# ZHANGKEON/DIS-YOLO

Hardware: AMD Instinct MI355X
Metric: train images/sec @576x576 bf16 (higher is better)
Workload: dtype bf16

## Files before the change

dis-yolo_amd/csrc/conv_igemm.hip:

```cpp
#include <utility>
#include "common.h"
#include "conv_common.h"
#include "runtime.h"

using namespace dyconv;

namespace {

template <int BM, int BN, int WM, int WN, int BK, int ST, int KS, int KG = 1, int EPI = 0>
__global__ __launch_bounds__(WM* WN * 64 * KG, (BM == 128 && BN == 128) ? 3 : 1) void conv_igemm_kernel(ConvParams p) {
#ifdef HALO_PROBE
  long long gp_t[5];
  gp_t[0] = (long long)__builtin_amdgcn_s_memtime();
  gp_t[4] = (long long)__builtin_amdgcn_s_memrealtime();
#endif
  constexpr int NW = WM * WN;
  constexpr int T = NW * 64;
  constexpr int WTM = BM / WM, WTN = BN / WN;
  constexpr int MI = WTM / 16, NI = WTN / 16;
  constexpr int ROWB = BK * 2;
  constexpr int CPR = ROWB / 16;
  constexpr int SLAB = 1024 * NW;
  constexpr int A_BYTES = (BM * ROWB + SLAB - 1) / SLAB * SLAB;
  constexpr int B_BYTES = (BN * ROWB + SLAB - 1) / SLAB * SLAB;
// ... 1421 lines not shown
          v[0] += __builtin_bit_cast(float, rr.x << 16);
          v[1] += __builtin_bit_cast(float, rr.x & 0xffff0000u);
          v[2] += __builtin_bit_cast(float, rr.y << 16);
          v[3] += __builtin_bit_cast(float, rr.y & 0xffff0000u);
        }
        uint2 o2;
        o2.x = pack2(v[0], v[1]);
        o2.y = pack2(v[2], v[3]);
        *reinterpret_cast<uint2*>(sw + (t * 16 + frow) * ROWP + (j * 16 + cq * 4) * 2) = o2;
      }
    }
    __builtin_amdgcn_fence(__ATOMIC_RELEASE, "wavefront");
    __builtin_amdgcn_wave_barrier();
    __builtin_amdgcn_fence(__ATOMIC_ACQUIRE, "wavefront");
#pragma unroll
    for (int t = 0; t < FW; ++t) {
#pragma unroll
      for (int r_ = 0; r_ < RPF; ++r_) {
        const int idx = r_ * 64 + lane;
        const int r16 = idx / CPR8, ch = idx % CPR8;
        const int m = __shfl(m_of[t], r16, 64);
        const int n = n0 + ch * 8;
        const uint4 o = *reinterpret_cast<const uint4*>(sw + (t * 16 + r16) * ROWP + ch * 16);
        unsigned off = (m >= 0 && n < p.Cout) ? (unsigned)(((size_t)m * p.Cout + n) * 2) : OOB;
#ifdef DY_PROBE
        if (p.flags & 0x80000) off = OOB;
#endif
        buffer_store16(o, off, srdy);
      }
    }
  }
}

template <int NI>
__global__ __launch_bounds__(512) void conv1x1_stream_kernel(ConvParams p, int ngroups) {
  constexpr int NW = 8, U = 2;
  constexpr int BN = NI * 16;
  constexpr int ROWP = BN * 2 + 16;
  constexpr int STG = U * 16 * ROWP;
  constexpr int MAXKS = 6;
  extern __shared__ __attribute__((aligned(16))) char smem[];
  const int tid = threadIdx.x;
  const int lane = tid & 63;
  const int wave = __builtin_amdgcn_readfirstlane(tid >> 6);
  const int frow = lane & 15, cq = lane >> 4;
  const int K = p.K, ks32 = K >> 5;
  const int wpitch = K * 2 + 16;
  char* const wl = smem;
  char* const stg = smem + ((BN * wpitch + 15) & ~15);
  for (int c = tid; c < BN * (K >> 3); c += NW * 64) {
    const int n = c / (K >> 3), kc = c - n * (K >> 3);
    uint4 v = uint4{0, 0, 0, 0};
    if (n < p.Cout) v = *reinterpret_cast<const uint4*>(p.w + (size_t)n * K + kc * 8);
    *reinterpret_cast<uint4*>(wl + n * wpitch + kc * 16) = v;
  }
  float esc[NI][4], esh[NI][4];
#pragma unroll
  for (int j = 0; j < NI; ++j)
#pragma unroll
    for (int r = 0; r < 4; ++r) {
      const int n = j * 16 + cq * 4 + r;
      esc[j][r] = (p.scale && n < p.Cout) ? p.scale[n] : 1.f;
      esh[j][r] = (p.shift && n < p.Cout) ? p.shift[n] : 0.f;
    }
  __syncthreads();
  const bool f32out = p.flags & DISYOLO_CONV_OUT_F32;
  const bool do_stats = p.flags & DISYOLO_CONV_STATS;
  const bool vec_ok = (p.Cout & 7) == 0;
  const bool use_res = p.residual != nullptr;
  const int H1 = p.H >> 1, W1 = p.W >> 1;
  const int ks0 = p.C0 >> 5;
  float s1[NI][4], s2[NI][4];
#pragma unroll
  for (int j = 0; j < NI; ++j)
#pragma unroll
    for (int r = 0; r < 4; ++r) s1[j][r] = s2[j][r] = 0.f;
  char* const sw = stg + wave * STG;

  for (int g = blockIdx.x * NW + wave; g < ngroups; g += gridDim.x * NW) {
    int m_of[U];
    bf16x8 xf[U][MAXKS];
#pragma unroll
    for (int u = 0; u < U; ++u) {
      const int m = g * (U * 16) + u * 16 + frow;
      m_of[u] = m < p.M ? m : -1;
      const int mm = m < p.M ? m : 0;
      const bf16* a0 = p.x0 + (size_t)mm * p.C0 + cq * 8;
      const bf16* a1 = a0;
      if (p.C1 > 0) {
        int b, rem, y, x;
        divmod_small(mm, p.H * p.W, b, rem);
        divmod_small(rem, p.W, y, x);
        a1 = p.x1 + ((size_t)(b * H1 + (y >> 1)) * W1 + (x >> 1)) * p.C1 + cq * 8;
      }
#pragma unroll
      for (int k = 0; k < MAXKS; ++k)
        if (k < ks32) xf[u][k] = *reinterpret_cast<const bf16x8*>(k < ks0 ? a0 + k * 32 : a1 + (k - ks0) * 32);
    }
    uint2 rres[U][NI];
    if (use_res) {
#pragma unroll
      for (int u = 0; u < U; ++u)
#pragma unroll
        for (int j = 0; j < NI; ++j) {
          const int n = j * 16 + cq * 4;
          rres[u][j] = *reinterpret_cast<const uint2*>(p.residual + (size_t)(m_of[u] >= 0 ? m_of[u] : 0) * p.Cout + (n + 3 < p.Cout ? n : 0));
        }
    }
    f32x4 acc[U][NI];
#pragma unroll
    for (int u = 0; u < U; ++u)
#pragma unroll
      for (int j = 0; j < NI; ++j) acc[u][j] = f32x4{0.f, 0.f, 0.f, 0.f};
#pragma unroll
    for (int k = 0; k < MAXKS; ++k) {
      if (k < ks32) {
        bf16x8 wf[NI];
#pragma unroll
        for (int j = 0; j < NI; ++j) wf[j] = *reinterpret_cast<const bf16x8*>(wl + (j * 16 + frow) * wpitch + (k * 4 + cq) * 16);
#pragma unroll
        for (int u = 0; u < U; ++u)
#pragma unroll
          for (int j = 0; j < NI; ++j) acc[u][j] = __builtin_amdgcn_mfma_f32_16x16x32_bf16(wf[j], xf[u][k], acc[u][j], 0, 0, 0);
      }
    }
    if (do_stats) {
#pragma unroll
      for (int u = 0; u < U; ++u)
#pragma unroll
        for (int j = 0; j < NI; ++j)
// ... 155 lines not shown
  static bool attr_set = false;
  if (!attr_set) {
    (void)hipFuncSetAttribute(reinterpret_cast<const void*>(&conv_stream_kernel<NW, FW, NI>),
                              hipFuncAttributeMaxDynamicSharedMemorySize, (int)lds);
    attr_set = true;
  }
  static const int ncu = [] {
    int dev = 0, n = 256;
    if (hipGetDevice(&dev) == hipSuccess) (void)hipDeviceGetAttribute(&n, hipDeviceAttributeMultiprocessorCount, dev);
    return n > 0 ? n : 256;
  }();
  int G = ncu / q.tilesN;
  if (G < 1) G = 1;
  if (G > q.tilesM) G = q.tilesM;
  hipLaunchKernelGGL((conv_stream_kernel<NW, FW, NI>), dim3(G * q.tilesN), dim3(NW * 64), lds, s, q, pt.ph, pt.pw, tilesY,
                     tilesX, G);
  DY_CHECK_LAUNCH();
  return DISYOLO_OK;
}

bool stream1x1_ok(const disyolo_conv_desc* d) {
  if (d->ksize != 1 || d->stride != 1 || d->in_div != 1 || d->Ho != d->H || d->Wo != d->W) return false;
  if (d->Cout > 64 || d->C0 % 32 || d->C1 % 32 || d->C0 + d->C1 > 192) return false;
  if (d->flags & DISYOLO_CONV_BN_BWD_STATS) return false;
  return true;
}
int stream1x1_blocks(int M) {
  const int groups = ceil_div(M, 32);
  int blocks = ceil_div(groups, 8 * 4);
  if (blocks > 512) blocks = 512;
  if (blocks < 1) blocks = 1;
  return blocks;
}
template <int NI>
int launch_stream1x1_n(const ConvParams& p, hipStream_t s) {
  constexpr int BN = NI * 16;
  const size_t wbytes = ((size_t)BN * (p.K * 2 + 16) + 15) & ~(size_t)15;
  const size_t lds = wbytes + (size_t)8 * 2 * 16 * (BN * 2 + 16) + (size_t)8 * BN * 8;
  static bool attr_set = false;
  if (!attr_set) {
    (void)hipFuncSetAttribute(reinterpret_cast<const void*>(&conv1x1_stream_kernel<NI>), hipFuncAttributeMaxDynamicSharedMemorySize,
                              (int)(64 * (192 * 2 + 16) + 8 * 2 * 16 * (64 * 2 + 16) + 8 * 64 * 8));
    attr_set = true;
  }
  hipLaunchKernelGGL((conv1x1_stream_kernel<NI>), dim3(stream1x1_blocks(p.M)), dim3(512), lds, s, p, ceil_div(p.M, 32));
  DY_CHECK_LAUNCH();
  return DISYOLO_OK;
}
int launch_stream1x1(const ConvParams& p, hipStream_t s) {
  if (p.Cout <= 16) return launch_stream1x1_n<1>(p, s);
  if (p.Cout <= 32) return launch_stream1x1_n<2>(p, s);
  return launch_stream1x1_n<4>(p, s);
}

struct LaunchQuery {
  bool active = false, have = false, want_bwd = false, want_fused = false;
  int grid = 0, rows = 0, bn = 0, resident = 0;
};
thread_local LaunchQuery tl_query;
template <class K>
int resident_blocks(K kernel, int threads, size_t lds) {
  int dev = 0, cus = 0, occ = 0;
  if (hipGetDevice(&dev) != hipSuccess) return 0;
  if (hipDeviceGetAttribute(&cus, hipDeviceAttributeMultiprocessorCount, dev) != hipSuccess) return 0;
  if (hipOccupancyMaxActiveBlocksPerMultiprocessor(&occ, reinterpret_cast<const void*>(kernel), threads, lds) != hipSuccess) {
    (void)hipGetLastError();
    return 0;
  }
  const int by_lds = lds ? (int)((size_t)160 * 1024 / lds) : 8;
  const int by_waves = 32 / (threads / 64);
  if (occ > by_lds) occ = by_lds;
  if (occ > by_waves) occ = by_waves;
  return occ * cus;
}

template <int NW, int FW, int NI>
int launch_halo(const ConvParams& p, Patch pt, hipStream_t s) {
  ConvParams q = p;
  constexpr int BN = NI * 16;
  const int tilesY = p.H / pt.ph, tilesX = p.W / pt.pw;
  q.tilesM = p.B * tilesY * tilesX;
  q.tilesN = ceil_div(p.Cout, BN);
  q.xcd_n = (q.tilesN >= 8 && (int64_t)p.bytesw > (int64_t)p.bytes0) ? 1 : 0;
  q.halo_split = 1;
  constexpr int SLAB = NW * 1024, BIM = (9 * BN * 4 + NW * 64 - 1) / (NW * 64);
// ... 364 lines not shown
extern "C" int disyolo_dgrad_s2_quad_ok(int B, int Hdy, int Wdy, int Cdy, int C) {
  return (B > 0 && Hdy > 0 && Wdy > 0 && Cdy % 64 == 0 && C % 8 == 0 && (4 * C) % 128 == 0 && C <= 64 &&
          (int64_t)B * Hdy * Wdy * 4 * C * 2 < (1LL << 31) && (int64_t)B * Hdy * Wdy * Cdy * 2 < (1LL << 31)) ? 1 : 0;
}

extern "C" int disyolo_dgrad_s2_quad(const void* dy, const void* wq, void* dx, const void* residual, int B, int Hdy, int Wdy,
                                     int Cdy, int C, void* stream) {
  DY_REQUIRE(dy && wq && dx, "dgrad_s2_quad: null pointer");
  DY_REQUIRE(disyolo_dgrad_s2_quad_ok(B, Hdy, Wdy, Cdy, C) == 1, "dgrad_s2_quad: needs Cdy %% 64 == 0, C in {32, 64}");
  DY_RECORD_OR_RUN([=](void* s) { return disyolo_dgrad_s2_quad(dy, wq, dx, residual, B, Hdy, Wdy, Cdy, C, s); });
  ConvParams p;
  p.x0 = (const bf16*)dy; p.x1 = nullptr; p.w = (const bf16*)wq;
  p.scale = nullptr; p.shift = nullptr; p.residual = (const bf16*)residual; p.y = dx; p.stats = nullptr;
  p.bn_x = nullptr; p.bn_scale = p.bn_shift = p.bn_mean = p.bn_rstd = nullptr; p.bn_part = nullptr; p.bn_alpha = 0.f;
  p.B = B; p.H = Hdy; p.W = Wdy; p.C0 = Cdy; p.C1 = 0; p.Cin = Cdy;
  p.Ho = Hdy; p.Wo = Wdy; p.Cout = 4 * C;
  p.ks = 3; p.stride = 1; p.pad_t = 1; p.pad_l = 1; p.dmask = 0; p.dshift = 0;
  p.M = B * Hdy * Wdy;
  p.K = 9 * Cdy;
  p.bytes0 = (unsigned)((size_t)B * Hdy * Wdy * Cdy * 2);
  p.bytes1 = 0;
  p.bytesw = (unsigned)((size_t)4 * C * 9 * Cdy * 2);
  p.nk = 0;
  p.flags = 0;
  p.alpha = 0.f;
  p.tilesM = p.tilesN = 0;
  p.xcd_n = 0; p.halo_split = 0;
  p.pcls = 0; p.Mc = 0; p.tilesMc = 0;
  p.tapmask = 0x1b;
  p.d2s_c = C;
  return launch<192, 128, 4, 2, 64, 2>(p, (hipStream_t)stream);
}

static int conv2d_fwd_core(const disyolo_conv_desc* d, void* stream);

extern "C" int disyolo_cluster_sync_words(int Cout) { return Cout > 0 ? (ceil_div(Cout, 16) + 1) * CL_LINE : 0; }

extern "C" int disyolo_cluster_sync_error(const uint32_t* cluster_sync, int Cout) {
  if (!cluster_sync || Cout <= 0) return 0;
  uint32_t w = 0;
  if (hipMemcpy(&w, cluster_sync + (size_t)ceil_div(Cout, 16) * CL_LINE, sizeof(w), hipMemcpyDeviceToHost) != hipSuccess) {
    (void)hipGetLastError();
    return -1;
  }
  return (int)w;
}

extern "C" int disyolo_conv2d_bn_fused_ok(const disyolo_conv_desc* d) {
  if (!d || validate(d) != DISYOLO_OK) return 0;
  if ((d->flags & DISYOLO_CONV_OUT_F32) || d->Cout % 8) return 0;
  if (d->in_div != 1 && (d->flags & (DISYOLO_CONV_STATS | DISYOLO_CONV_BN_FUSED))) return 0;
  static const bool on = [] { const char* e = getenv("DISYOLO_BN_INKERNEL"); return !(e && e[0] == '0'); }();
  if (!on) return 0;
  tl_query = LaunchQuery{};
  tl_query.active = true;
  tl_query.want_bwd = (d->flags & DISYOLO_CONV_BN_BWD_FUSED) != 0;
  tl_query.want_fused = true;
  disyolo_conv_desc c = *d;
  c.flags &= ~(DISYOLO_CONV_BN_FUSED | DISYOLO_CONV_BN_BWD_FUSED | DISYOLO_CONV_BN_BWD_STATS);
  const int rc = conv2d_fwd_core(&c, nullptr);
  const LaunchQuery q = tl_query;
  tl_query = LaunchQuery{};
  if (rc != DISYOLO_OK || !q.have) return 0;
  if ((int64_t)q.rows * q.bn * 8 > 128 * 1024) return 0;
  return (q.resident > 0 && q.grid <= q.resident) ? 1 : 0;
}

extern "C" int disyolo_conv2d_fwd(const disyolo_conv_desc* d, void* stream) {
  int rc = validate(d);
  if (rc) return rc;
  DY_REQUIRE(!(d->flags & DISYOLO_CONV_STATS) || d->stats, "conv: STATS flag without stats buffer");
  if (d->flags & DISYOLO_CONV_BN_FUSED) {
    DY_REQUIRE((d->flags & DISYOLO_CONV_STATS) && !(d->flags & (DISYOLO_CONV_LEAKY | DISYOLO_CONV_OUT_F32 | DISYOLO_CONV_BN_BWD_STATS)) &&
                   !d->scale && !d->shift && !d->residual && d->Cout % 8 == 0,
               "conv: BN_FUSED needs STATS, bf16 y, no scale / shift / LEAKY / residual (y is the raw conv output), Cout %% 8 == 0");
    DY_REQUIRE(d->y_act && d->bn_gamma && d->bn_beta && d->bn_out_scale && d->bn_out_shift && d->bn_out_mean && d->bn_out_rstd &&
                   d->cluster_sync, "conv: BN_FUSED with a null y_act / bn_gamma / bn_beta / bn_out_* / cluster_sync");
  }
  if (d->flags & DISYOLO_CONV_BN_BWD_FUSED) {
    DY_REQUIRE((d->flags & DISYOLO_CONV_BN_BWD_STATS) && d->bn_dgamma && d->bn_dbeta && d->cluster_sync,
               "conv: BN_BWD_FUSED needs BN_BWD_STATS (the bn_* fields) and bn_dgamma / bn_dbeta / cluster_sync");
  }
  {
    const disyolo_conv_desc c = *d;
    DY_RECORD_OR_RUN([c](void* s) { return disyolo_conv2d_fwd(&c, s); });
  }
  return conv2d_fwd_core(d, stream);
}

static int conv2d_fwd_core(const disyolo_conv_desc* d, void* stream) {
  if (conv_c16_shape(d)) {
    if (tl_query.active) return DISYOLO_OK;
    return conv_c16_launch(d, stream);
  }
  ConvParams p;
  p.x0 = (const bf16*)d->x0;
  p.x1 = (const bf16*)d->x1;
  p.w = (const bf16*)d->w;
  p.scale = d->scale;
  p.shift = d->shift;
  p.residual = (const bf16*)d->residual;
  p.y = d->y;
  p.stats = d->stats;
  p.bn_x = nullptr; p.bn_scale = p.bn_shift = p.bn_mean = p.bn_rstd = nullptr; p.bn_part = nullptr; p.bn_alpha = 0.f;
  if (d->flags & DISYOLO_CONV_BN_BWD_STATS) {
    DY_REQUIRE(d->bn_x && d->bn_scale && d->bn_shift && d->bn_mean && d->bn_rstd && d->bn_partials,
               "conv: BN_BWD_STATS flag with a null bn_* pointer");
    DY_REQUIRE((d->flags & DISYOLO_CONV_BN_BWD_FUSED) || disyolo_conv2d_bn_bwd_stats_ok(d) == 1,
               "conv: BN_BWD_STATS needs a patch kernel (tile 16-19, 24, 25 on a shape it covers) or a GEMM tile with that epilogue "
               "(ask disyolo_conv2d_bn_bwd_stats_ok), bf16 output, Cout %% 8 == 0");
    DY_REQUIRE(!(d->flags & DISYOLO_CONV_BN_BWD_FUSED) || (!(d->flags & (DISYOLO_CONV_OUT_F32 | DISYOLO_CONV_STATS | DISYOLO_CONV_LEAKY)) &&
                                                          !d->scale && !d->shift && d->Cout % 8 == 0),
               "conv: BN_BWD_FUSED needs a plain bf16 data-gradient conv (no scale / shift / LEAKY / STATS), Cout %% 8 == 0");
    p.bn_x = (const bf16*)d->bn_x; p.bn_scale = d->bn_scale; p.bn_shift = d->bn_shift; p.bn_mean = d->bn_mean;
    p.bn_rstd = d->bn_rstd; p.bn_part = d->bn_partials; p.bn_alpha = d->bn_alpha;
  }
  p.B = d->B; p.H = d->H; p.W = d->W; p.C0 = d->C0; p.C1 = d->C1; p.Cin = d->C0 + d->C1;
  p.Ho = d->Ho; p.Wo = d->Wo; p.Cout = d->Cout;
  p.ks = d->ksize; p.stride = d->stride; p.pad_t = d->pad_t; p.pad_l = d->pad_l;
  p.dmask = d->in_div - 1; p.dshift = d->in_div == 2 ? 1 : 0;
  p.M = d->B * d->Ho * d->Wo;
  p.K = d->ksize * d->ksize * p.Cin;
  p.bytes0 = (unsigned)((size_t)d->B * d->H * d->W * d->C0 * 2);
  p.bytes1 = (unsigned)((size_t)d->B * (d->H / 2) * (d->W / 2) * d->C1 * 2);
  p.bytesw = (unsigned)((size_t)d->Cout * p.K * 2);
  p.nk = 0;
  p.flags = d->flags;
  p.alpha = d->alpha;
  p.tilesM = p.tilesN = 0;
  p.xcd_n = 0; p.halo_split = 0;
  p.pcls = 0; p.Mc = 0; p.tilesMc = 0;
  p.tapmask = 0; p.d2s_c = 0;
  p.y_act = d->y_act; p.gamma = d->bn_gamma; p.beta = d->bn_beta; p.mm = d->bn_moving_mean; p.mv = d->bn_moving_var;
  p.o_scale = d->bn_out_scale; p.o_shift = d->bn_out_shift; p.o_mean = d->bn_out_mean; p.o_rstd = d->bn_out_rstd;
  p.dgamma = d->bn_dgamma; p.dbeta = d->bn_dbeta; p.csync = d->cluster_sync;
  p.bn_decay = d->bn_decay; p.bn_eps = d->bn_eps; p.inv_count = 1.0 / (double)p.M;
  hipStream_t s = (hipStream_t)stream;
  Patch pt;
  const int sel = resolve_sel(d, p.M, &pt);
  {
    const int id = sel & 0xff;
    if (id == 24 || id == 25 || id == 20 || id == 21) {
      if (tl_query.active) return DISYOLO_OK;
      DY_REQUIRE(!(d->flags & (DISYOLO_CONV_BN_FUSED | DISYOLO_CONV_BN_BWD_FUSED)),
                 "conv: BN_FUSED / BN_BWD_FUSED on a tile whose kernel has no such epilogue (ask disyolo_conv2d_bn_fused_ok)");
    }
  }
  switch (sel & 0xff) {
    case 24:
    case 25: return launch_flat(p, sel & 0xff, s);
#ifndef DY_ONLY_HALO
    case 21: return launch_stream1x1(p, s);
    case 20: return launch_stream(p, pt, s);
#endif
    case 16: return launch_halo<8, 3, 4>(p, pt, s);
    case 18: return launch_halo<8, 3, 2>(p, pt, s);
    case 19: return launch_halo<8, 3, 1>(p, pt, s);
    case 17: return launch_halo<4, 3, 4>(p, pt, s);
    default: break;
  }
  const bool bk64 = (d->C0 % 64 == 0) && (d->C1 % 64 == 0) && !(sel & 0x100);
  return dispatch(sel & 0xff, bk64, (sel >> 9) & 1, p, s);
}
```

dis-yolo_amd/lib.py:

```python
from __future__ import annotations

import ctypes as C
import os
from typing import Optional

import numpy as np
import torch

_HERE = os.path.dirname(os.path.abspath(__file__))
LIB_PATH = os.environ.get("DISYOLO_LIB", os.path.join(_HERE, "libdisyolo_hip.so"))

GRAD_LD = 32
ROI_MAX = 16
ROI_W = 12
K_MAPS = (3, 5, 7)
MASK_STRIDES = (1, 2, 4)


def roi_w(k: int) -> int:
    return 2 * (k + 1) + 4


def block32_post(k: int) -> int:
    return {3: 1, 5: 2, 7: 3}[k]
# ... 8 lines not shown
    _fields_ = [
        ("B", C.c_int32), ("H", C.c_int32), ("W", C.c_int32),
        ("C0", C.c_int32), ("C1", C.c_int32),
        ("Ho", C.c_int32), ("Wo", C.c_int32), ("Cout", C.c_int32),
        ("ksize", C.c_int32), ("stride", C.c_int32),
        ("pad_t", C.c_int32), ("pad_l", C.c_int32),
        ("in_div", C.c_int32), ("flags", C.c_int32),
        ("alpha", C.c_float), ("tile", C.c_int32),
        ("x0", C.c_void_p), ("x1", C.c_void_p), ("w", C.c_void_p),
        ("scale", C.c_void_p), ("shift", C.c_void_p), ("residual", C.c_void_p),
        ("y", C.c_void_p), ("stats", C.c_void_p),
        ("bn_x", C.c_void_p), ("bn_scale", C.c_void_p), ("bn_shift", C.c_void_p), ("bn_mean", C.c_void_p),
        ("bn_rstd", C.c_void_p), ("bn_partials", C.c_void_p), ("bn_alpha", C.c_float),
        ("bn_decay", C.c_float), ("bn_eps", C.c_float),
        ("y_act", C.c_void_p), ("bn_gamma", C.c_void_p), ("bn_beta", C.c_void_p),
        ("bn_moving_mean", C.c_void_p), ("bn_moving_var", C.c_void_p),
        ("bn_out_scale", C.c_void_p), ("bn_out_shift", C.c_void_p), ("bn_out_mean", C.c_void_p), ("bn_out_rstd", C.c_void_p),
        ("bn_dgamma", C.c_void_p), ("bn_dbeta", C.c_void_p), ("cluster_sync", C.c_void_p),
    ]


_SIGS = {
    "disyolo_version": (C.c_int, []),
    "disyolo_last_error": (C.c_char_p, []),
    "disyolo_conv_desc_size": (C.c_size_t, []),
    "disyolo_find_contours": (C.c_int, [C.c_void_p, C.c_int, C.c_int, C.c_void_p, C.c_int64, C.c_void_p, C.c_void_p, C.c_int,
                                        C.POINTER(C.c_int), C.POINTER(C.c_int64)]),
    "disyolo_conv2d_stats_rows": (C.c_int, [C.POINTER(ConvDesc)]),
    "disyolo_conv2d_bn_bwd_stats_ok": (C.c_int, [C.POINTER(ConvDesc)]),
    "disyolo_conv2d_bn_fused_ok": (C.c_int, [C.POINTER(ConvDesc)]),
    "disyolo_cluster_sync_words": (C.c_int, [C.c_int]),
    "disyolo_cluster_sync_error": (C.c_int, [C.c_void_p, C.c_int]),
    "disyolo_conv2d_fwd": (C.c_int, [C.POINTER(ConvDesc), C.c_void_p]),
    "disyolo_conv2d_tile": (C.c_int, [C.POINTER(ConvDesc)] + [C.POINTER(C.c_int)] * 4),
    "disyolo_conv_first_fwd": (C.c_int, [C.c_void_p] * 5 + [C.c_int] * 4 + [C.c_float, C.c_void_p]),
    "disyolo_conv12_fused_ok": (C.c_int, [C.c_int] * 3),
    "disyolo_conv12_fused_fwd": (C.c_int, [C.c_void_p] * 8 + [C.c_int] * 3 + [C.c_float, C.c_void_p]),
    "disyolo_block32_fused_ok": (C.c_int, [C.c_int] * 6),
    "disyolo_block64_fused_ok": (C.c_int, [C.c_int] * 4),
    "disyolo_pack_quad": (C.c_int, [C.c_void_p, C.c_void_p, C.c_int, C.c_int, C.c_void_p]),
    "disyolo_dgrad_s2_quad_ok": (C.c_int, [C.c_int] * 5),
    "disyolo_dgrad_s2_quad": (C.c_int, [C.c_void_p] * 4 + [C.c_int] * 5 + [C.c_void_p]),
    "disyolo_block64_fused_fwd": (C.c_int, [C.c_void_p] * 8 + [C.c_int] * 4 + [C.c_float, C.c_void_p]),
    "disyolo_block32_fused_fwd": (C.c_int, [C.c_void_p, C.c_void_p, C.c_int, C.c_int] + [C.c_void_p] * 6 + [C.c_int] +
                                  [C.c_void_p] * 3 + [C.c_int] * 3 + [C.c_float, C.c_void_p]),
    "disyolo_conv2d_wgrad_workspace": (C.c_size_t, [C.POINTER(ConvDesc), C.c_int]),
    "disyolo_conv2d_wgrad": (C.c_int, [C.POINTER(ConvDesc), C.c_void_p, C.c_int, C.c_void_p, C.c_void_p,
                                       C.c_size_t, C.c_int, C.c_void_p]),
    "disyolo_conv2d_fp8_fwd": (C.c_int, [C.POINTER(ConvDesc), C.c_void_p, C.c_void_p, C.c_void_p, C.c_void_p, C.c_float,
                                         C.c_void_p, C.c_float, C.c_void_p, C.c_void_p]),
    "disyolo_conv_first_fwd_fp8": (C.c_int, [C.c_void_p] * 5 + [C.c_float] + [C.c_int] * 4 + [C.c_float, C.c_void_p]),
    "disyolo_quant_fp8": (C.c_int, [C.c_void_p, C.c_int, C.c_void_p, C.c_int64, C.c_float, C.c_void_p]),
    "disyolo_dequant_fp8": (C.c_int, [C.c_void_p, C.c_void_p, C.c_int64, C.c_float, C.c_void_p]),
    "disyolo_pack_weights_fp8": (C.c_int, [C.c_void_p, C.c_void_p] + [C.c_int] * 3 + [C.c_float, C.c_void_p]),
    "disyolo_conv2d_wgrad_plan": (C.c_int, [C.POINTER(ConvDesc), C.c_int] + [C.POINTER(C.c_int)] * 4),
    "disyolo_conv_first_wgrad_workspace": (C.c_size_t, [C.c_int] * 4),
    "disyolo_conv_first_wgrad": (C.c_int, [C.c_void_p] * 3 + [C.c_int] * 4 + [C.c_void_p, C.c_size_t, C.c_void_p]),
    "disyolo_image_pad8": (C.c_int, [C.c_void_p, C.c_void_p, C.c_int64, C.c_void_p]),
    "disyolo_copy2d_f32": (C.c_int, [C.c_void_p, C.c_void_p] + [C.c_int] * 4 + [C.c_void_p]),
    "disyolo_pack_weights": (C.c_int, [C.c_void_p] * 3 + [C.c_int] * 4 + [C.c_void_p]),
    "disyolo_pack_table_bytes": (C.c_size_t, [C.c_int]),
    "disyolo_pack_table_build": (C.c_int, [C.c_void_p, C.c_int, C.c_void_p, C.POINTER(C.c_int)]),
    "disyolo_pack_all": (C.c_int, [C.c_void_p, C.c_int, C.c_int, C.c_void_p]),
    "disyolo_bn_finalize": (C.c_int, [C.c_void_p, C.c_int, C.c_int, C.c_int64] + [C.c_void_p] * 4 +
                            [C.c_float, C.c_float] + [C.c_void_p] * 5),
    "disyolo_colstats_rows": (C.c_int, [C.c_int64, C.c_int]),
# ... 406 lines not shown
def conv2d_tile(d: ConvDesc):
    bm, bn, bk, st = C.c_int(0), C.c_int(0), C.c_int(0), C.c_int(0)
    tid = load().disyolo_conv2d_tile(C.byref(d), C.byref(bm), C.byref(bn), C.byref(bk), C.byref(st))
    if tid < 0:
        raise DisyoloError("conv2d_tile: bad descriptor")
    return tid, bm.value, bn.value, bk.value, st.value


def conv2d_fwd(d: ConvDesc) -> None:
    if TUNER is not None:
        TUNER.launch(d)
        return
    if TIMER is not None:
        if not hasattr(d, "_tname"):
            tid, bm, bn, bk, st = conv2d_tile(d)
            if tid in (24, 25):
                d._tname = "conv_flat_kernel<%s,2,%d>" % ("2,3,2,1" if tid == 24 else "4,3,1,2", st)
            elif tid == 21:
                d._tname = "conv1x1_stream_kernel<%d>" % (bn // 16)
            elif tid == 20:
                d._tname = "conv_stream_kernel<8,3,4>"
            elif tid >= 16:
                d._tname = "conv_halo_kernel<%d,3,%d>" % (4 if tid == 17 else 8, 2 if tid == 18 else 1 if tid == 19 else 4)
            else:
                d._tname = "conv_igemm_kernel<%d,%d,%d,%d,%d,%d,%d,%d,%d>" % ((bm, bn) + _WAVES.get(tid, (0, 0)) +
                                                                               (bk, st, d.ksize, 2 if 13 <= tid <= 15 else 1,
                                                                                1 if d.flags & CONV_BN_BWD_FUSED else 0))
        TIMER.run(d._tname, conv_flops(d), lambda: _check(load().disyolo_conv2d_fwd(C.byref(d), _stream()),
                                                           "conv2d_fwd"), conv_bytes(d))
        return
    _check(load().disyolo_conv2d_fwd(C.byref(d), _stream()), "conv2d_fwd")


def conv2d_fp8_fwd(d: ConvDesc, w8, escale, eshift, y8, out_scale: float, y16=None, residual8=None,
                   residual_scale: float = 0.0) -> None:
    if TIMER is not None:
        name = "conv_fp8_kernel<%d,%d,3>" % (128 if d.Cout > 64 else (64 if d.Cout > 32 else 32), 64 if d.C0 % 64 == 0 else 32)
        TIMER.run(name, conv_flops(d), lambda: _check(load().disyolo_conv2d_fp8_fwd(
            C.byref(d), _p(w8), _p(escale), _p(eshift), _p(residual8), residual_scale, _p(y8), out_scale, _p(y16), _stream()),
            "conv2d_fp8_fwd"))
        return
    _check(load().disyolo_conv2d_fp8_fwd(C.byref(d), _p(w8), _p(escale), _p(eshift), _p(residual8), residual_scale, _p(y8),
                                         out_scale, _p(y16), _stream()), "conv2d_fp8_fwd")


def conv_first_fwd_fp8(images, w_hwio, scale, shift, y8, out_scale: float, alpha=0.1) -> None:
    _need(images, torch.float32, "images")
    _need(y8, torch.uint8, "y8")
    B, H, W, _ = images.shape
    _check(load().disyolo_conv_first_fwd_fp8(_p(images), _p(w_hwio), _p(scale), _p(shift), _p(y8), out_scale, B, H, W,
                                             y8.shape[-1], alpha, _stream()), "conv_first_fwd_fp8")


def quant_fp8(x, y8, scale: float) -> None:
    if x.dtype not in (torch.bfloat16, torch.float32) or not x.is_contiguous():
        raise DisyoloError("quant_fp8: x must be contiguous bf16 or f32")
    _check(load().disyolo_quant_fp8(_p(x), int(x.dtype == torch.float32), _p(y8), x.numel(), scale, _stream()), "quant_fp8")


def dequant_fp8(x8, y, scale: float) -> None:
    _need(y, torch.float32, "y")
    _check(load().disyolo_dequant_fp8(_p(x8), _p(y), x8.numel(), scale, _stream()), "dequant_fp8")


def pack_weights_fp8(w_hwio, w8, ksize, cin, cout, scale: float) -> None:
    _check(load().disyolo_pack_weights_fp8(_p(w_hwio), _p(w8), ksize, cin, cout, scale, _stream()), "pack_weights_fp8")
# ... 595 lines not shown
```

dis-yolo_amd/net.py:

```python
from __future__ import annotations

from typing import Dict, List, Optional, Sequence, Tuple

import math
import json
import contextlib
import os
import sys
import numpy as np
import torch

from . import config as cfg
from . import lib as L

BF16 = torch.bfloat16
F32 = torch.float32

WGRAD_GROUP = 3
OPT_CHUNK_ELEMS = 8_000_000
PIPE_LANE = 2


class Layer:
    __slots__ = ("idx", "cin", "cout", "k", "stride", "kind", "src", "src_up", "shortcut", "lock", "H", "W", "Ho",
                 "Wo", "w", "bias", "gamma", "beta", "mm", "mv", "scale", "shift", "mean", "rstd", "wp", "wdg", "raw",
                 "act", "stats", "stats_rows", "desc", "grad", "grad_set", "need_grad", "dw", "dbias", "dgamma",
                 "dbeta", "dx", "pad_t", "pad_l", "dgrad_descs", "wgrad_desc", "cout_pad",
                 "act8", "w8", "s_w", "s_out", "escale", "desc8", "dual16", "bn_sums", "bwd_local", "bwd_global", "bwd_part", "bwd_part_rows", "wq",
                 "csync", "fused_fwd", "csync_bwd", "fused_bwd", "passthru")

    def __init__(self, idx, cin, cout, k, stride, kind, src, src_up=None, shortcut=None):
        self.idx, self.cin, self.cout, self.k, self.stride, self.kind = idx, cin, cout, k, stride, kind
        self.src, self.src_up, self.shortcut = src, src_up, shortcut
        for s in self.__slots__[9:]:
            setattr(self, s, None)


MASK_STRIDES = (4, 2, 1)


def build_topology(num_class: int, k_map: int, mask_stride: int = 2) -> List[Layer]:
    if mask_stride not in MASK_STRIDES:
        raise ValueError("mask_stride must be one of %s (got %r)" % (", ".join(map(str, MASK_STRIDES)), mask_stride))
    out_depth = (num_class + 5) * 3
    Ls: List[Layer] = []

    def add(idx, cin, cout, k, s, kind, src, src_up=None, shortcut=None):
        Ls.append(Layer(idx, cin, cout, k, s, kind, src, src_up, shortcut))

    add(1, 3, 32, 3, 1, "bn", 0)
    add(2, 32, 64, 3, 2, "bn", 1)
    i = 3
    ch = 64
    for nblocks, down in ((1, 5), (2, 10), (8, 27), (8, 44), (4, None)):
        for _ in range(nblocks):
            add(i, ch, ch // 2, 1, 1, "bn", i - 1)
            add(i + 1, ch // 2, ch, 3, 1, "res", i, shortcut=i - 1)
            i += 2
        if down:
            add(down, ch, ch * 2, 3, 2, "bn", down - 1)
            ch *= 2
            i = down + 1
# ... 99 lines not shown
            self.ws = L.Workspace(self.device)
            self.ws_aux = L.Workspace(self.device)
            self.ws_det = L.Workspace(self.device)
        self._reg_fresh = False
        self.lock = {i: (stage == 1 and i <= 52) for i in range(1, self.score_layer + 1)}
        for i, v in (lock or {}).items():
            if isinstance(i, bool) or not isinstance(i, (int, np.integer)) or not 1 <= i <= self.score_layer:
                raise ValueError("lock: %r is not a layer of this net (1..%d)" % (i, self.score_layer))
            self.lock[int(i)] = bool(v)
        self.layers = build_topology(self.num_class, self.k, self.mask_stride)
        self.by_idx = {l.idx: l for l in self.layers}
        self._mark_pass_through()
        if self.dtype == "fp8":
            self._check_fp8_lock()
        self._lr = float(cfg.LEARNING_RATE)
        self.lr_dev = None
        self.dp = None
        self.sync_bn = False
        self._rec = None
        self._prog = None
        self._prog_marks = []
        self._graph = None
        self.opt_chunks = None
        self._overlap = False
        self._overlap_rec = False
        self._tail_open = False
        self._progs = None
        self.fuse_first_two = True
        self.fuse_blocks = True
        self.use_side_lane = os.environ.get("DISYOLO_SIDE_LANE", "1") != "0"
        self.bn_inkernel = os.environ.get("DISYOLO_BN_INKERNEL", "1") != "0"
        self.bn_inkernel_bwd = os.environ.get("DISYOLO_BN_INKERNEL_BWD", "0") == "1"
        self.bn_fuse_check = None
        self.tail_on_main = 0
        self.pair = bool(backbone_pair)
        self._half = 0
        self._pair_P = 0
        self._init_params(seed, xavier_locked)
        if self.pair:
            if not self.training or self.dtype != "bf16" or self.plan_only:
                raise L.DisyoloError("backbone_pair needs a bf16 training net")
            self._pair_P = self._backbone_prefix()
            if self._pair_P < 2:
                raise L.DisyoloError("backbone_pair needs a locked layer prefix (stage 1)")
        if not self.plan_only:
            self._plan(self.batchsize, self.image_size)

    def _init_params(self, seed: int, xavier_locked: bool) -> None:
        dev = self.device
        g = torch.Generator().manual_seed(seed)
        n_decay = 0
        n_nodecay = 0
        for l in self.layers:
            l.lock = self.lock[l.idx]
            if not l.lock:
                n_decay += l.k * l.k * l.cin * l.cout + (l.cout if l.kind == "lin" else 0)
                if l.kind != "lin":
                    n_nodecay += 2 * l.cout
        self.n_decay, self.n_params = n_decay, n_decay + n_nodecay
        n = max(self.n_params, 1)
        self.arena = torch.zeros(n, dtype=F32, device=dev)
        self.grad_arena = torch.zeros(n, dtype=F32, device=dev)
        self.adam_m = torch.zeros(n, dtype=F32, device=dev)
        self.adam_v = torch.zeros(n, dtype=F32, device=dev)
        self.step_dev = torch.zeros(1, dtype=torch.int64, device=dev)
        self.lr_dev = torch.full((1,), self._lr, dtype=F32, device=dev)
# ... 283 lines not shown
            if l.kind == "lin":
                l.desc = L.make_conv_desc(x0, l.wp, l.act, l.k, l.stride, x1=x1, shift=l.bias, out_f32=True)
            elif train_bn:
                if l.stats is None:
                    d0 = L.make_conv_desc(x0, l.wp, l.raw, l.k, l.stride, x1=x1)
                    l.stats_rows = L.conv2d_stats_rows(d0)
                    l.stats = torch.zeros(l.stats_rows, l.cout, 2, dtype=F32, device=dev)
                l.desc = L.make_conv_desc(x0, l.wp, l.raw, l.k, l.stride, x1=x1, stats=l.stats)
                l.fused_fwd = False
                if (self.bn_inkernel and not self.sync_bn and res is None and l.idx not in self.HEAD_LAYERS
                        and not getattr(self, "plan_only", False) and l.stride == 1):
                    tile = self._fused_tile(lambda t: L.make_conv_desc(x0, l.wp, l.raw, l.k, l.stride, x1=x1, tile=t), l.k)
                    if tile is not None:
                        d0 = L.make_conv_desc(x0, l.wp, l.raw, l.k, l.stride, x1=x1, tile=tile)
                        rows = L.conv2d_stats_rows(d0)
                        l.stats_rows = rows
                        if l.stats.shape[0] < rows:
                            l.stats = torch.zeros(rows, l.cout, 2, dtype=F32, device=dev)
                        if l.csync is None:
                            l.csync = L.cluster_sync_buffer(l.cout, dev)
                        l.desc = L.make_conv_desc(x0, l.wp, l.raw, l.k, l.stride, x1=x1, stats=l.stats, tile=tile,
                                                  bn_fused=dict(y_act=l.act, gamma=l.gamma, beta=l.beta, mm=l.mm, mv=l.mv,
                                                                scale=l.scale, shift=l.shift, mean=l.mean, rstd=l.rstd,
                                                                decay=cfg.BN_DECAY, eps=cfg.BN_EPSILON, sync=l.csync),
                                                  alpha=cfg.ALPHA)
                        l.fused_fwd = True
            elif l.passthru:
                l.desc = L.make_conv_desc(x0, l.wp, l.raw, l.k, l.stride, x1=x1)
            else:
                l.desc = L.make_conv_desc(x0, l.wp, l.act, l.k, l.stride, x1=x1, scale=l.scale, shift=l.shift,
                                          residual=res, leaky=True, alpha=cfg.ALPHA)
            if self.training and not l.lock:
                l.wgrad_desc = L.make_conv_desc(x0, l.wp, l.act, l.k, l.stride, x1=x1)

    FUSED_TILES_1x1 = (3, 2, 6, 10, 1, 12, 0x20c)
    FUSED_TILES_3x3 = (16, 18, 19, 12, 0x20c)

    def _fused_tile(self, make_desc, k: int, bwd: bool = False):
        best, best_blocks = None, -1
        for i, t in enumerate((0,) + (self.FUSED_TILES_3x3 if k == 3 else self.FUSED_TILES_1x1)):
            d = make_desc(t)
            tid, bm, bn, _, _ = L.conv2d_tile(d)
            if t and tid != (t & 0xff):
                continue
            if bwd:
                d.flags |= L.CONV_BN_BWD_FUSED
            ok = L.conv2d_bn_fused_ok(d)
            d.flags &= ~L.CONV_BN_BWD_FUSED
            if not ok:
                continue
            if i == 0:
                return d.tile
            blocks = L.conv2d_stats_rows(d) * (-(-d.Cout // bn))
            if blocks > best_blocks:
                best, best_blocks = t, blocks
        return best

    def _input_of(self, l, src: int) -> torch.Tensor:
        a = self.by_idx[src].act
        if self.pair and src <= self._pair_P < l.idx:
            return a[self._half * self.B:(self._half + 1) * self.B]
        return a

    def _backbone_prefix(self) -> int:
        p = 0
        for l in self.layers:
# ... 262 lines not shown
                    and L.block32_fused_ok(self.B, l82.Ho, l82.Wo, self.by_idx[l80.src].cout, self.by_idx[l80.src_up].cout,
                                           L.block32_post(self.k))):
                plan[80], plan[81], plan[82] = None, None, self._forward_mask_head
        return plan

    def _can_fuse_first_two(self, is_training: bool) -> bool:
        if not self.fuse_first_two or (self.dtype == "fp8" and self.fp8_ready and self.FP8_FROM <= 2):
            return False
        if not self._inference_mode((1, 2), is_training):
            return False
        if any(1 in (l.src, l.src_up, l.shortcut) for l in self.layers if l.idx != 2):
            return False
        return L.conv12_fused_ok(self.B, self.S, self.S)

    def _forward_layer(self, l, is_training: bool) -> None:
        B = self.B
        if self.dtype == "fp8" and self.fp8_ready and l.act8 is not None and l.idx >= self.FP8_FROM:
            self._forward_layer_fp8(l)
            return
        train_bn = is_training and self.training and (not l.lock) and l.kind != "lin"
        M = B * l.Ho * l.Wo
        res = self._input_of(l, l.shortcut) if l.shortcut is not None else None
        if l.idx == 1:
            if train_bn:
                L.conv_first_fwd(self.images, l.w, self._ones32, self._zeros32, l.raw, alpha=1.0)
                L.colstats(l.raw, l.stats, M, l.cout)
                self._bn_finalize(l, M)
                L.bn_act_fwd(l.raw, l.scale, l.shift, None, l.act, M, l.cout, cfg.ALPHA)
            else:
                if not l.lock and self.training:
                    L.bn_fold(l.gamma, l.beta, l.mm, l.mv, cfg.BN_EPSILON, l.scale, l.shift)
                L.conv_first_fwd(self.images, l.w, l.scale, l.shift, l.act, alpha=cfg.ALPHA)
            return
        if l.kind == "lin":
            L.conv2d_fwd(l.desc)
        elif l.passthru and is_training:
            L.conv2d_fwd(l.desc)
            L.bn_act_fwd(l.raw, l.scale, l.shift, res, l.act, M, l.cout, cfg.ALPHA)
        elif train_bn:
            L.conv2d_fwd(l.desc)
            if l.fused_fwd and L.TUNER is None:
                return
            self._bn_finalize(l, M)
            L.bn_act_fwd(l.raw, l.scale, l.shift, res, l.act, M, l.cout, cfg.ALPHA)
        else:
            if self.training and (not l.lock or l.passthru):
                if not l.lock:
                    L.bn_fold(l.gamma, l.beta, l.mm, l.mv, cfg.BN_EPSILON, l.scale, l.shift)
                d = L.make_conv_desc(self._input_of(l, l.src), l.wp, l.act, l.k, l.stride,
                                     x1=self._input_of(l, l.src_up) if l.src_up is not None else None,
                                     scale=l.scale, shift=l.shift, residual=res, leaky=True, alpha=cfg.ALPHA)
                L.conv2d_fwd(d)
            else:
                L.conv2d_fwd(l.desc)

    def _bn_finalize(self, l, M: int) -> None:
        rows = l.stats_rows
        if L.TUNER is not None:
            rows = L.TUNER.stats_rows.get(l.stats.data_ptr(), rows)
        if not self.sync_bn:
            L.bn_finalize(l.stats, rows, l.cout, M, l.gamma, l.beta, l.mm, l.mv, cfg.BN_DECAY,
                          cfg.BN_EPSILON, l.scale, l.shift, l.mean, l.rstd)
            return
        L.bn_partial_sums(l.stats, rows, l.cout, l.bn_sums)
        self._sync_sums(l.bn_sums)
        L.bn_finalize_sums(l.bn_sums, l.cout, M * self.dp.world_size, l.gamma, l.beta, l.mm, l.mv, cfg.BN_DECAY,
                           cfg.BN_EPSILON, l.scale, l.shift, l.mean, l.rstd)

    def _sync_sums(self, t: torch.Tensor) -> None:
        if self.dp.inlist:
            self.dp.comm.allreduce(t)
        elif self._rec is not None:
            prog, marks = self._rec
            marks.append((prog.size(), ("sync", t, L.CURRENT_LANE)))
        else:
            import torch.distributed as dist
# ... 826 lines not shown
```

include/disyolo.h:

```cpp
#ifndef DISYOLO_H
#define DISYOLO_H

#include <stddef.h>
#include <stdint.h>

#ifdef __cplusplus
extern "C" {
#endif

#define DISYOLO_OK 0
#define DISYOLO_E_ARG (-1)
#define DISYOLO_E_WORKSPACE (-2)
#define DISYOLO_E_HIP (-3)

#define DISYOLO_GRAD_LD 32
#define DISYOLO_ROI_MAX 16
#define DISYOLO_ROI_W 12
#define DISYOLO_ROI_W_K(k) (2 * ((k) + 1) + 4)

int disyolo_version(void);
const char* disyolo_last_error(void);

enum {
  DISYOLO_CONV_LEAKY = 1,
// ... 24 lines not shown
  float* stats;
  const void* bn_x;
  const float* bn_scale;
  const float* bn_shift;
  const float* bn_mean;
  const float* bn_rstd;
  float* bn_partials;
  float bn_alpha;
  float bn_decay, bn_eps;
  void* y_act;
  const float* bn_gamma;
  const float* bn_beta;
  float* bn_moving_mean;
  float* bn_moving_var;
  float* bn_out_scale;
  float* bn_out_shift;
  float* bn_out_mean;
  float* bn_out_rstd;
  float* bn_dgamma;
  float* bn_dbeta;
  uint32_t* cluster_sync;
} disyolo_conv_desc;

int disyolo_find_contours(const uint8_t* binary, int h, int w, int32_t* points_xy, int64_t max_points,
                          int32_t* contour_start, int32_t* hierarchy, int max_contours, int* n_contours,
                          int64_t* n_points);
size_t disyolo_conv_desc_size(void);
int disyolo_conv2d_bn_bwd_stats_ok(const disyolo_conv_desc* d);
int disyolo_conv2d_bn_fused_ok(const disyolo_conv_desc* d);
int disyolo_cluster_sync_words(int Cout);
int disyolo_cluster_sync_error(const uint32_t* cluster_sync, int Cout);
int disyolo_conv2d_stats_rows(const disyolo_conv_desc* d);
int disyolo_conv2d_fwd(const disyolo_conv_desc* d, void* stream);
int disyolo_conv2d_tile(const disyolo_conv_desc* d, int* bm, int* bn, int* bk, int* stages);

int disyolo_conv_first_fwd(const float* images, const float* w_hwio, const float* scale,
                           const float* shift, void* y_bf16, int B, int H, int W, int Cout,
                           float alpha, void* stream);

int disyolo_conv12_fused_ok(int B, int H, int W);
int disyolo_conv12_fused_fwd(const float* images, const float* w1_hwio, const float* scale1, const float* shift1,
                             const void* w2_packed, const float* scale2, const float* shift2, void* y_bf16, int B, int H,
                             int W, float alpha, void* stream);

int disyolo_block32_fused_ok(int B, int H, int W, int C0, int C1, int post);
int disyolo_block32_fused_fwd(const void* x0, const void* x1, int C0, int C1, const void* wA, const float* scaleA,
                              const float* shiftA, const void* wB, const float* scaleB, const float* shiftB, int post,
                              const void* wC, const float* biasC, void* y, int B, int H, int W, float alpha, void* stream);

int disyolo_block64_fused_ok(int B, int H, int W, int C0);
int disyolo_block64_fused_fwd(const void* x, const void* wA, const float* scaleA, const float* shiftA, const void* wB,
                              const float* scaleB, const float* shiftB, void* y, int B, int H, int W, int C0, float alpha,
                              void* stream);

int disyolo_pack_quad(const float* w_hwio, void* wq, int C, int Cdy, void* stream);
int disyolo_dgrad_s2_quad_ok(int B, int Hdy, int Wdy, int Cdy, int C);
int disyolo_dgrad_s2_quad(const void* dy, const void* wq, void* dx, const void* residual, int B, int Hdy, int Wdy, int Cdy,
                          int C, void* stream);

enum {
  DISYOLO_WGRAD_IM2COL = 1,
  DISYOLO_WGRAD_PARTIAL_ONLY = 2,
  DISYOLO_WGRAD_REDUCE_ONLY = 4,
  DISYOLO_WGRAD_STAGES_MASK = 0x30
};
size_t disyolo_conv2d_wgrad_workspace(const disyolo_conv_desc* d, int opts);
// ... 218 lines not shown
```

Measured before the change: 2148.

## Fuse producer BN+leaky activation into streaming 1x1 conv input load

Adds a BNL variant of the streaming 1x1 conv kernel. It reads the producer layer's raw pre-BN output, applies the producer's batch-norm scale/shift and leaky activation on load, and writes the activated tensor out for backward use. The network planner finds eligible producer→1x1 consumer pairs and skips the separate bn_act_fwd launch for those producers. This removes a kernel launch and one read of the raw tensor per pair. In exchange the consumer kernel does extra ALU work, extra stores and a little more LDS.

```diff
diff --git a/dis-yolo_amd/csrc/conv_igemm.hip b/dis-yolo_amd/csrc/conv_igemm.hip
--- a/dis-yolo_amd/csrc/conv_igemm.hip
+++ b/dis-yolo_amd/csrc/conv_igemm.hip
@@ -1477,7 +1477,7 @@
   }
 }
 
-template <int NI>
+template <int NI, bool BNL = false>
 __global__ __launch_bounds__(512) void conv1x1_stream_kernel(ConvParams p, int ngroups) {
   constexpr int NW = 8, U = 2;
   constexpr int BN = NI * 16;
@@ -1499,6 +1499,13 @@
     if (n < p.Cout) v = *reinterpret_cast<const uint4*>(p.w + (size_t)n * K + kc * 8);
     *reinterpret_cast<uint4*>(wl + n * wpitch + kc * 16) = v;
   }
+  float* const isc = reinterpret_cast<float*>(stg + NW * STG + NW * BN * 8);
+  if (BNL) {
+    for (int c = tid; c < p.C0; c += NW * 64) {
+      isc[c] = p.bn_scale[c];
+      isc[p.C0 + c] = p.bn_shift[c];
+    }
+  }
   float esc[NI][4], esh[NI][4];
 #pragma unroll
   for (int j = 0; j < NI; ++j)
@@ -1541,6 +1548,28 @@
 #pragma unroll
       for (int k = 0; k < MAXKS; ++k)
         if (k < ks32) xf[u][k] = *reinterpret_cast<const bf16x8*>(k < ks0 ? a0 + k * 32 : a1 + (k - ks0) * 32);
+    }
+    if (BNL) {
+#pragma unroll
+      for (int k = 0; k < MAXKS; ++k) {
+        if (k < ks32) {
+          const int c0 = k * 32 + cq * 8;
+          const float4 s0 = *reinterpret_cast<const float4*>(isc + c0), s1 = *reinterpret_cast<const float4*>(isc + c0 + 4);
+          const float4 h0 = *reinterpret_cast<const float4*>(isc + p.C0 + c0), h1 = *reinterpret_cast<const float4*>(isc + p.C0 + c0 + 4);
+          const float sc[8] = {s0.x, s0.y, s0.z, s0.w, s1.x, s1.y, s1.z, s1.w};
+          const float sh[8] = {h0.x, h0.y, h0.z, h0.w, h1.x, h1.y, h1.z, h1.w};
+#pragma unroll
+          for (int u = 0; u < U; ++u) {
+            float v[8];
+            unpack8(__builtin_bit_cast(uint4, xf[u][k]), v);
+#pragma unroll
+            for (int e = 0; e < 8; ++e) v[e] = leaky(v[e] * sc[e] + sh[e], p.bn_alpha);
+            const uint4 o = pack8(v);
+            xf[u][k] = __builtin_bit_cast(bf16x8, o);
+            if (m_of[u] >= 0) *reinterpret_cast<uint4*>(reinterpret_cast<bf16*>(p.y_act) + (size_t)m_of[u] * p.C0 + c0) = o;
+          }
+        }
+      }
     }
     uint2 rres[U][NI];
     if (use_res) {
@@ -1762,25 +1791,26 @@
   if (blocks < 1) blocks = 1;
   return blocks;
 }
-template <int NI>
+template <int NI, bool BNL = false>
 int launch_stream1x1_n(const ConvParams& p, hipStream_t s) {
   constexpr int BN = NI * 16;
   const size_t wbytes = ((size_t)BN * (p.K * 2 + 16) + 15) & ~(size_t)15;
-  const size_t lds = wbytes + (size_t)8 * 2 * 16 * (BN * 2 + 16) + (size_t)8 * BN * 8;
+  const size_t lds = wbytes + (size_t)8 * 2 * 16 * (BN * 2 + 16) + (size_t)8 * BN * 8 + (BNL ? (size_t)p.C0 * 8 : 0);
   static bool attr_set = false;
   if (!attr_set) {
-    (void)hipFuncSetAttribute(reinterpret_cast<const void*>(&conv1x1_stream_kernel<NI>), hipFuncAttributeMaxDynamicSharedMemorySize,
-                              (int)(64 * (192 * 2 + 16) + 8 * 2 * 16 * (64 * 2 + 16) + 8 * 64 * 8));
+    (void)hipFuncSetAttribute(reinterpret_cast<const void*>(&conv1x1_stream_kernel<NI, BNL>), hipFuncAttributeMaxDynamicSharedMemorySize,
+                              (int)(64 * (192 * 2 + 16) + 8 * 2 * 16 * (64 * 2 + 16) + 8 * 64 * 8 + 192 * 8));
     attr_set = true;
   }
-  hipLaunchKernelGGL((conv1x1_stream_kernel<NI>), dim3(stream1x1_blocks(p.M)), dim3(512), lds, s, p, ceil_div(p.M, 32));
+  hipLaunchKernelGGL((conv1x1_stream_kernel<NI, BNL>), dim3(stream1x1_blocks(p.M)), dim3(512), lds, s, p, ceil_div(p.M, 32));
   DY_CHECK_LAUNCH();
   return DISYOLO_OK;
 }
+template <bool BNL = false>
 int launch_stream1x1(const ConvParams& p, hipStream_t s) {
-  if (p.Cout <= 16) return launch_stream1x1_n<1>(p, s);
-  if (p.Cout <= 32) return launch_stream1x1_n<2>(p, s);
-  return launch_stream1x1_n<4>(p, s);
+  if (p.Cout <= 16) return launch_stream1x1_n<1, BNL>(p, s);
+  if (p.Cout <= 32) return launch_stream1x1_n<2, BNL>(p, s);
+  return launch_stream1x1_n<4, BNL>(p, s);
 }
 
 struct LaunchQuery {
@@ -2211,7 +2241,13 @@
   return launch<192, 128, 4, 2, 64, 2>(p, (hipStream_t)stream);
 }
 
-static int conv2d_fwd_core(const disyolo_conv_desc* d, void* stream);
+struct BnInput {
+  const float* scale;
+  const float* shift;
+  void* act;
+  float alpha;
+};
+static int conv2d_fwd_core(const disyolo_conv_desc* d, void* stream, const BnInput* bn_in = nullptr);
 
 extern "C" int disyolo_cluster_sync_words(int Cout) { return Cout > 0 ? (ceil_div(Cout, 16) + 1) * CL_LINE : 0; }
 
@@ -2267,7 +2303,31 @@
   return conv2d_fwd_core(d, stream);
 }
 
-static int conv2d_fwd_core(const disyolo_conv_desc* d, void* stream) {
+extern "C" int disyolo_conv1x1_bn_in_fwd_ok(const disyolo_conv_desc* d) {
+  if (!d || validate(d) != DISYOLO_OK || conv_c16_shape(d)) return 0;
+  if (d->C1 != 0 || (d->flags & (DISYOLO_CONV_BN_FUSED | DISYOLO_CONV_BN_BWD_FUSED | DISYOLO_CONV_BN_BWD_STATS))) return 0;
+  return (resolve_sel(d, d->B * d->Ho * d->Wo, nullptr) & 0xff) == 21 ? 1 : 0;
+}
+
+extern "C" int disyolo_conv1x1_bn_in_fwd(const disyolo_conv_desc* d, const float* in_scale, const float* in_shift, void* in_act,
+                                         float in_alpha, void* stream) {
+  int rc = validate(d);
+  if (rc) return rc;
+  DY_REQUIRE(in_scale && in_shift && in_act, "conv1x1_bn_in_fwd: null in_scale / in_shift / in_act");
+  DY_REQUIRE(in_act != d->x0 && in_act != d->y, "conv1x1_bn_in_fwd: in_act aliases x0 or y");
+  DY_REQUIRE(!(d->flags & DISYOLO_CONV_STATS) || d->stats, "conv: STATS flag without stats buffer");
+  DY_REQUIRE(disyolo_conv1x1_bn_in_fwd_ok(d) == 1,
+             "conv1x1_bn_in_fwd: needs the streaming 1x1 kernel (tile 21 on a shape it covers), one source (C1 == 0), no in-launch "
+             "batch norm (ask disyolo_conv1x1_bn_in_fwd_ok)");
+  {
+    const disyolo_conv_desc c = *d;
+    DY_RECORD_OR_RUN([=](void* s) { return disyolo_conv1x1_bn_in_fwd(&c, in_scale, in_shift, in_act, in_alpha, s); });
+  }
+  const BnInput bi{in_scale, in_shift, in_act, in_alpha};
+  return conv2d_fwd_core(d, stream, &bi);
+}
+
+static int conv2d_fwd_core(const disyolo_conv_desc* d, void* stream, const BnInput* bn_in) {
   if (conv_c16_shape(d)) {
     if (tl_query.active) return DISYOLO_OK;
     return conv_c16_launch(d, stream);
@@ -2329,7 +2389,12 @@
     case 24:
     case 25: return launch_flat(p, sel & 0xff, s);
 #ifndef DY_ONLY_HALO
-    case 21: return launch_stream1x1(p, s);
+    case 21:
+      if (bn_in) {
+        p.bn_scale = bn_in->scale; p.bn_shift = bn_in->shift; p.bn_alpha = bn_in->alpha; p.y_act = bn_in->act;
+        return launch_stream1x1<true>(p, s);
+      }
+      return launch_stream1x1<false>(p, s);
     case 20: return launch_stream(p, pt, s);
 #endif
     case 16: return launch_halo<8, 3, 4>(p, pt, s);
diff --git a/dis-yolo_amd/lib.py b/dis-yolo_amd/lib.py
--- a/dis-yolo_amd/lib.py
+++ b/dis-yolo_amd/lib.py
@@ -64,6 +64,8 @@
     "disyolo_cluster_sync_words": (C.c_int, [C.c_int]),
     "disyolo_cluster_sync_error": (C.c_int, [C.c_void_p, C.c_int]),
     "disyolo_conv2d_fwd": (C.c_int, [C.POINTER(ConvDesc), C.c_void_p]),
+    "disyolo_conv1x1_bn_in_fwd_ok": (C.c_int, [C.POINTER(ConvDesc)]),
+    "disyolo_conv1x1_bn_in_fwd": (C.c_int, [C.POINTER(ConvDesc), C.c_void_p, C.c_void_p, C.c_void_p, C.c_float, C.c_void_p]),
     "disyolo_conv2d_tile": (C.c_int, [C.POINTER(ConvDesc)] + [C.POINTER(C.c_int)] * 4),
     "disyolo_conv_first_fwd": (C.c_int, [C.c_void_p] * 5 + [C.c_int] * 4 + [C.c_float, C.c_void_p]),
     "disyolo_conv12_fused_ok": (C.c_int, [C.c_int] * 3),
@@ -536,6 +538,27 @@
     _check(load().disyolo_conv2d_fwd(C.byref(d), _stream()), "conv2d_fwd")
 
 
+def conv1x1_bn_in_fwd_ok(d: ConvDesc) -> bool:
+    return load().disyolo_conv1x1_bn_in_fwd_ok(C.byref(d)) == 1
+
+
+def conv1x1_bn_in_fwd(d: ConvDesc, in_scale, in_shift, in_act, in_alpha=0.1) -> None:
+    _need(in_scale, torch.float32, "in_scale")
+    _need(in_shift, torch.float32, "in_shift")
+    _need(in_act, torch.bfloat16, "in_act")
+    if in_scale.numel() != d.C0 or in_shift.numel() != d.C0 or in_act.numel() != d.B * d.H * d.W * d.C0:
+        raise DisyoloError("conv1x1_bn_in_fwd: in_scale / in_shift / in_act do not match the descriptor's source 0")
+
+    def run():
+        _check(load().disyolo_conv1x1_bn_in_fwd(C.byref(d), _p(in_scale), _p(in_shift), _p(in_act), in_alpha, _stream()),
+               "conv1x1_bn_in_fwd")
+    if TIMER is not None:
+        nb = conv_bytes(d) + d.B * d.H * d.W * d.C0 * 2
+        TIMER.run("conv1x1_stream_kernel<%d,true>" % (1 if d.Cout <= 16 else 2 if d.Cout <= 32 else 4), conv_flops(d), run, nb)
+        return
+    run()
+
+
 def conv2d_fp8_fwd(d: ConvDesc, w8, escale, eshift, y8, out_scale: float, y16=None, residual8=None,
                    residual_scale: float = 0.0) -> None:
     if TIMER is not None:
diff --git a/dis-yolo_amd/net.py b/dis-yolo_amd/net.py
--- a/dis-yolo_amd/net.py
+++ b/dis-yolo_amd/net.py
@@ -27,7 +27,7 @@
                  "act", "stats", "stats_rows", "desc", "grad", "grad_set", "need_grad", "dw", "dbias", "dgamma",
                  "dbeta", "dx", "pad_t", "pad_l", "dgrad_descs", "wgrad_desc", "cout_pad",
                  "act8", "w8", "s_w", "s_out", "escale", "desc8", "dual16", "bn_sums", "bwd_local", "bwd_global", "bwd_part", "bwd_part_rows", "wq",
-                 "csync", "fused_fwd", "csync_bwd", "fused_bwd", "passthru")
+                 "csync", "fused_fwd", "csync_bwd", "fused_bwd", "passthru", "bn_in_desc", "act_by")
 
     def __init__(self, idx, cin, cout, k, stride, kind, src, src_up=None, shortcut=None):
         self.idx, self.cin, self.cout, self.k, self.stride, self.kind = idx, cin, cout, k, stride, kind
@@ -193,6 +193,7 @@
         self.bn_inkernel = os.environ.get("DISYOLO_BN_INKERNEL", "1") != "0"
         self.bn_inkernel_bwd = os.environ.get("DISYOLO_BN_INKERNEL_BWD", "0") == "1"
         self.bn_fuse_check = None
+        self.bn_on_load = True
         self.tail_on_main = 0
         self.pair = bool(backbone_pair)
         self._half = 0
@@ -542,6 +543,36 @@
                                           residual=res, leaky=True, alpha=cfg.ALPHA)
             if self.training and not l.lock:
                 l.wgrad_desc = L.make_conv_desc(x0, l.wp, l.act, l.k, l.stride, x1=x1)
+        self._plan_bn_on_load()
+
+    def _plan_bn_on_load(self) -> None:
+        for l in self.layers:
+            l.bn_in_desc, l.act_by = None, None
+        if not self.training or self.dtype == "fp8" or getattr(self, "plan_only", False):
+            return
+        for l in self.layers:
+            s = self.by_idx.get(l.src)
+            if s is None or s.idx == 1 or l.src_up is not None or l.shortcut is not None or l.lock or l.k != 1:
+                continue
+            if s.lock or s.kind == "lin" or s.raw is None or s.shortcut is not None or s.fused_fwd:
+                continue
+            if any(s.idx in (o.src, o.src_up, o.shortcut) for o in self.layers if o is not l):
+                continue
+            x0 = self._input_of(l, l.src)
+            if x0.data_ptr() != s.act.data_ptr() or x0.shape != s.act.shape or s.raw.shape != s.act.shape:
+                continue
+            if l.kind == "lin":
+                d = L.make_conv_desc(s.raw, l.wp, l.act, l.k, l.stride, shift=l.bias, out_f32=True, tile=l.desc.tile)
+            elif not l.fused_fwd:
+                d = L.make_conv_desc(s.raw, l.wp, l.raw, l.k, l.stride, stats=l.stats, tile=l.desc.tile)
+            else:
+                continue
+            if L.conv1x1_bn_in_fwd_ok(d):
+                l.bn_in_desc, s.act_by = d, l.idx
+
+    def _bn_on_load(self, l, is_training: bool) -> bool:
+        return (l.bn_in_desc is not None and self.bn_on_load and is_training and self.training and L.TUNER is None
+                and not (self.dtype == "fp8" and self.fp8_ready))
 
     FUSED_TILES_1x1 = (3, 2, 6, 10, 1, 12, 0x20c)
     FUSED_TILES_3x3 = (16, 18, 19, 12, 0x20c)
@@ -870,7 +901,14 @@
                     L.bn_fold(l.gamma, l.beta, l.mm, l.mv, cfg.BN_EPSILON, l.scale, l.shift)
                 L.conv_first_fwd(self.images, l.w, l.scale, l.shift, l.act, alpha=cfg.ALPHA)
             return
-        if l.kind == "lin":
+        if self._bn_on_load(l, is_training):
+            s = self.by_idx[l.src]
+            L.conv1x1_bn_in_fwd(l.bn_in_desc, s.scale, s.shift, s.act, cfg.ALPHA)
+            if l.kind != "lin":
+                self._bn_finalize(l, M)
+                if l.act_by is None or not self._bn_on_load(self.by_idx[l.act_by], is_training):
+                    L.bn_act_fwd(l.raw, l.scale, l.shift, res, l.act, M, l.cout, cfg.ALPHA)
+        elif l.kind == "lin":
             L.conv2d_fwd(l.desc)
         elif l.passthru and is_training:
             L.conv2d_fwd(l.desc)
@@ -880,6 +918,8 @@
             if l.fused_fwd and L.TUNER is None:
                 return
             self._bn_finalize(l, M)
+            if l.act_by is not None and self._bn_on_load(self.by_idx[l.act_by], is_training):
+                return
             L.bn_act_fwd(l.raw, l.scale, l.shift, res, l.act, M, l.cout, cfg.ALPHA)
         else:
             if self.training and (not l.lock or l.passthru):
diff --git a/include/disyolo.h b/include/disyolo.h
--- a/include/disyolo.h
+++ b/include/disyolo.h
@@ -80,6 +80,9 @@
 int disyolo_cluster_sync_error(const uint32_t* cluster_sync, int Cout);
 int disyolo_conv2d_stats_rows(const disyolo_conv_desc* d);
 int disyolo_conv2d_fwd(const disyolo_conv_desc* d, void* stream);
+int disyolo_conv1x1_bn_in_fwd_ok(const disyolo_conv_desc* d);
+int disyolo_conv1x1_bn_in_fwd(const disyolo_conv_desc* d, const float* in_scale, const float* in_shift, void* in_act,
+                              float in_alpha, void* stream);
 int disyolo_conv2d_tile(const disyolo_conv_desc* d, int* bm, int* bn, int* bk, int* stages);
 
 int disyolo_conv_first_fwd(const float* images, const float* w_hwio, const float* scale,
```

New measurement: 2144. No clear change (-0.2%).
